# MatchaChoco010/toy-cpu-pathtracing

Measured on AMD Instinct MI355X. Metric: Msamples/sec (whole node), scene3 MIS/Sobol 1920x1080, higher is better.
Workload: dtype f32; 1 GPU; scene3 1920x1080 mis+sobol, 1024-spp job, 1024 sample indices per step (BASELINE configs[1]); parallelism=single-gpu

## Files before the change

include/mi355pt_debug.h:

```cpp
#ifndef MI355PT_DEBUG_H
#define MI355PT_DEBUG_H
#include "mi355pt.h"
#ifdef __cplusplus
extern "C" {
#endif

int mi355pt_debug_unlock(int on);

int mi355pt_scene_debug_set_lowering(mi355pt_scene* s, int mode);

int mi355pt_scene_debug_lowering_digest(const mi355pt_scene* s, const mi355pt_camera* cam, char* names_buf, size_t names_len,
                                        uint64_t* digests, uint32_t* n);

int mi355pt_scene_export_bvh(const mi355pt_scene* s, void* out_nodes, uint32_t* n_nodes, void* out_tris, uint32_t* n_tris,
                             int32_t* root);
int mi355pt_probe_bvh_collapse(const float* tri_pos, uint32_t n_tris, const float* rays_od, uint32_t n_rays, uint32_t* out_info,
                               uint32_t* out_mismatch);
int mi355pt_probe_bvh_collapse_nodes(const void* bvh2_nodes, uint32_t n_nodes, int32_t root, uint32_t n_tris, uint32_t* out_info );
int mi355pt_probe_sobol(uint32_t width, uint32_t height, uint32_t spp, uint32_t seed, const uint32_t* xys ,
                        uint32_t n, const char* pattern, uint32_t* out_bits );
int mi355pt_probe_sincos(uint32_t first_bits, uint32_t stride, uint32_t n, uint64_t* out_counts );
int mi355pt_probe_intersect(const mi355pt_scene* s, const float* origins, const float* dirs, uint32_t n, float* out_t,
                            uint32_t* out_instance, uint32_t* out_triangle, float* out_normal );
int mi355pt_probe_occluded(const mi355pt_scene* s, const float* origins, const float* dirs, const float* t_max, uint32_t n,
                           uint8_t* out_hit);
int mi355pt_sample_log_records(const mi355pt_camera* cam, const mi355pt_params* p, uint32_t sample_begin, uint32_t sample_end,
                               size_t* out_records);
int mi355pt_render_sample_log(const mi355pt_scene* s, const mi355pt_camera* cam, const mi355pt_params* p, uint32_t sample_begin,
                              uint32_t sample_end, float* out_L, float* out_lambda, float* out_pdf, size_t n_records,
                              float* out_accum);
int mi355pt_probe_radiance(const mi355pt_scene* s, const mi355pt_camera* cam, const mi355pt_params* p, const uint32_t* xys,
                           uint32_t n, float* out_L, float* out_lambda, float* out_pdf);


#ifdef __cplusplus
// ... 4 lines not shown
```

toy-cpu-pathtracing_amd/csrc/api.cpp:

```cpp
#include <hip/hip_runtime.h>

#include <algorithm>
#include <cmath>
#include <cstdio>
#include <cstring>
#include <string>
#include <vector>

#include "../../include/mi355pt.h"
#include "api_internal.hpp"

using namespace pt;

static thread_local std::string g_err;
bool pt::g_debug_unlocked = false;
int pt::fail(int code, const std::string& msg) { g_err = msg; return code; }

static const uint32_t CIE_CMF_BITS[470 * 4] = {
#include "cie_cmf.inc"
};
void pt::cie_cmf4(float out[470 * 4]) { std::memcpy(out, CIE_CMF_BITS, sizeof(CIE_CMF_BITS)); }

namespace {

// ... 91 lines not shown
    LaunchCtx* lc; int slot;
    if ((rc = get_launch_ctx(s, p->seed, &lc, &slot))) return rc;
    if (lc->device != s->impl.device) return fail(MI355PT_E_DEVICE, "launch context and scene live on different devices");
    const bool want_stats = stats && p->collect_stats;
    int& waves = aov ? lc->aov_waves[aov_kind] : lc->waves[want_stats ? 1 : 0][p->sampler & 1u][p->strategy < 3u ? p->strategy : 0u];
    if (!waves) waves = aov ? query_resident_waves_aov((uint32_t)aov_kind, s->impl.features)
                            : query_resident_waves(select_kernel(false, want_stats, s->impl.features, p->sampler, p->strategy));
    const DevCamera dc = make_camera(cam);
    LaunchPlan plan = d_list ? plan_launch_tiles(cam, p, s_begin, s_end, waves, n_list) : plan_launch(cam, p, s_begin, s_end, waves, aov);
    DevParams& dp = plan.params;
    if (d_list) set_tile_list(dp, d_list);
    unsigned* d_counter = lc->d_counters + slot;
    DevStats* d_stats = lc->d_stats + slot;
    HIP_TRY(hipMemsetAsync(d_counter, 0, sizeof(unsigned), stream));
    dp.stats_mode = p->collect_stats;
    if (want_stats || (aov && stats)) HIP_TRY(hipMemsetAsync(d_stats, 0, sizeof(DevStats), stream));
    hipEvent_t e0 = nullptr, e1 = nullptr;
    if (stats) { HIP_TRY(hipEventCreate(&e0)); HIP_TRY(hipEventCreate(&e1)); HIP_TRY(hipEventRecord(e0, stream)); }
    if ((rc = grow_device_buffer(&lc->d_partial, &lc->partial_bytes, plan.partial_floats * sizeof(float), stream))) return rc;
    const KernelKey key = select_kernel(d_list != nullptr, want_stats, s->impl.features, p->sampler, p->strategy);
    if ((rc = grow_device_buffer(&lc->d_defer, &lc->defer_bytes, aov ? (size_t)0 : query_defer_bytes_per_wave(key) * (size_t)plan.grid, stream))) return rc;
    if (aov) HIP_TRY(launch_aov((uint32_t)aov_kind, s->impl.dev, dc, dp, illuminant_lut, lc->d_hash, d_accum, d_counter, stats ? d_stats : nullptr,
                                s->impl.features, plan.grid, stream));
    else HIP_TRY(launch_pt(key, s->impl.dev, dc, dp, plan.n_tiles,
                           lc->d_hash, d_accum, lc->d_partial, d_counter, d_list ? nullptr : d_stats, plan.grid, stream, pout, lc->d_defer));
    if (stats) {
        HIP_TRY(hipEventRecord(e1, stream));
        HIP_TRY(hipEventSynchronize(e1));
        float ms = 0.0f;
        HIP_TRY(hipEventElapsedTime(&ms, e0, e1));
        std::memset(stats, 0, sizeof(*stats));
        stats->kernel_ms = ms; stats->launches = 1;
        if (want_stats || aov) {
            DevStats h;
            HIP_TRY(hipMemcpy(&h, d_stats, sizeof(h), hipMemcpyDeviceToHost));
            copy_stats(h, stats);
        }
        (void)hipEventDestroy(e0); (void)hipEventDestroy(e1);
    }
    return MI355PT_OK;
}

static int launch_ranges(const mi355pt_scene* s, const mi355pt_camera* cam, const mi355pt_params* p, uint32_t s_begin, uint32_t s_end, float* d_accum,
                         hipStream_t stream, mi355pt_stats* stats, const uint32_t* d_list, uint32_t n_list,
                         const PathOut& pout = PathOut{nullptr, nullptr, nullptr, 0u, 0u}, int aov_kind = -1, uint32_t illuminant_lut = 0) {
    return for_each_launch_range(p->sampler, stats != nullptr, s_begin, s_end, [&](uint32_t b, uint32_t e) {
        return launch_range(s, cam, p, b, e, d_accum, stream, stats, pout, aov_kind, illuminant_lut, d_list, n_list);
    });
// ... 720 lines not shown
```

toy-cpu-pathtracing_amd/csrc/api_debug.cpp:

```cpp
#include <hip/hip_runtime.h>

#include <algorithm>
#include <cmath>
#include <cstring>
#include <string>
#include <vector>

#include "../../include/mi355pt_debug.h"
#include "api_internal.hpp"
#include "scene_lower.hpp"

using namespace pt;

extern "C" {

int mi355pt_debug_unlock(int on) { const int was = g_debug_unlocked ? 1 : 0; g_debug_unlocked = on != 0; return was; }

int mi355pt_scene_debug_set_lowering(mi355pt_scene* s, int mode) {
    if (!s) return fail(MI355PT_E_INVALID, "null argument");
    if (mode < 0 || mode > 2) return fail(MI355PT_E_INVALID, "unknown lowering mode");
    s->impl.lowering = mode;
    return MI355PT_OK;
}

int mi355pt_scene_debug_lowering_digest(const mi355pt_scene* s, const mi355pt_camera* cam, char* names_buf, size_t names_len, uint64_t* digests, uint32_t* n) {
    if (!s || !cam || !names_buf || !digests || !n) return fail(MI355PT_E_INVALID, "null argument");
    std::string err;
    int rc;
    LoweredGeometry geo; BvhOut bvh; LoweredScene ls; LowerReport rep;
    if ((rc = lower_geometry(s->impl, cam, &geo, &err))) return fail(rc, err);
    build_bvh(geo.build_tris, &bvh);
    if (bvh.max_depth >= STACK_DEPTH) return fail(MI355PT_E_INVALID, "BVH deeper than the traversal stack");
    float cmf[470 * 4];
    cie_cmf4(cmf);
    if ((rc = lower_scene(s->impl, std::move(geo), std::move(bvh), cmf, &ls, &rep, &err)) || (rc = lower_tree4(&ls, &rep, &err))) return fail(rc, err);
    std::vector<std::string> names; std::vector<uint64_t> dig;
    lowering_digests(ls, rep, &names, &dig);
    std::string text;
    for (const std::string& nm : names) text += nm + "\n";
    text += lowering_info(ls, rep, false, nullptr);
    const uint32_t cap = *n;
    *n = (uint32_t)dig.size();
    if (cap < dig.size() || names_len < text.size() + 1) return fail(MI355PT_E_INVALID, "digest or name buffer too small");
    std::memcpy(digests, dig.data(), dig.size() * sizeof(uint64_t));
    std::memcpy(names_buf, text.c_str(), text.size() + 1);
    return MI355PT_OK;
}

int mi355pt_sample_log_records(const mi355pt_camera* cam, const mi355pt_params* p, uint32_t s_begin, uint32_t s_end, size_t* out_records) {
    if (!cam || !p || !out_records || s_end <= s_begin) return fail(MI355PT_E_INVALID, "bad argument");
    *out_records = (size_t)shard_tile_count(cam->width, cam->height, p->shard_index, p->shard_count) * 64u * (s_end - s_begin);
    return MI355PT_OK;
}

int mi355pt_render_sample_log(const mi355pt_scene* s, const mi355pt_camera* cam, const mi355pt_params* p, uint32_t s_begin, uint32_t s_end,
                              float* out_L, float* out_lambda, float* out_pdf, size_t n_records, float* out_accum) {
    int rc = check_args(s, cam, p);
    if (rc) return rc;
    if (!out_L || !out_lambda || !out_pdf || s_end > p->spp || s_begin >= s_end) return fail(MI355PT_E_INVALID, "bad sample range or null output");
    if (p->spp & (p->spp - 1u)) return fail(MI355PT_E_INVALID, "the per-sample log needs a power-of-two spp (the sample index is read back from the Morton index)");
    if (p->collect_stats) return fail(MI355PT_E_INVALID, "the per-sample log is written by the production kernel, not the instrumented one");
    const size_t need = (size_t)shard_tile_count(cam->width, cam->height, p->shard_index, p->shard_count) * 64u * (s_end - s_begin);
    if (n_records != need) return fail(MI355PT_E_INVALID, "n_records must be tiles of the shard * 64 * (sample_end - sample_begin)");
    if (need == 0) return MI355PT_OK;
    const size_t n_film = (size_t)cam->width * cam->height * 3;
    DevBuf<float> d_L, d_lam, d_pdf, d_acc;
    HIP_TRY(d_L.alloc(need * 4)); HIP_TRY(d_lam.alloc(need * 4)); HIP_TRY(d_pdf.alloc(need * 4)); HIP_TRY(d_acc.alloc(n_film));
    HIP_TRY(hipMemset(d_L.p, 0, need * 16)); HIP_TRY(hipMemset(d_lam.p, 0, need * 16)); HIP_TRY(hipMemset(d_pdf.p, 0, need * 16));
// ... 183 lines not shown
```

toy-cpu-pathtracing_amd/csrc/launch_plan.hpp:

```cpp
#pragma once
#include <algorithm>
#include <cmath>
#include <cstddef>
#include <cstdint>
#include <cstdlib>

#include "../../include/mi355pt.h"
#include "layout.hpp"

namespace pt {

struct V3 { float x, y, z; };
inline V3 cross3(V3 a, V3 b) { return {a.y * b.z - b.y * a.z, a.z * b.x - b.z * a.x, a.x * b.y - b.x * a.y}; }
inline V3 norm3(V3 a) { float r = 1.0f / std::sqrt((a.x * a.x) + (a.y * a.y) + (a.z * a.z)); return {a.x * r, a.y * r, a.z * r}; }

inline uint32_t log2_int(uint32_t v) { return v == 0 ? 0 : 31 - (uint32_t)__builtin_clz(v); }
inline uint32_t round_up_pow2(uint32_t v) { return v <= 1 ? 1 : 1u << (32 - __builtin_clz(v - 1)); }

inline uint32_t shard_tile_count(uint32_t width, uint32_t height, uint32_t shard_index, uint32_t shard_count) {
    const uint32_t total = ((width + 7) / 8) * ((height + 7) / 8);
    const uint32_t cnt = shard_count ? shard_count : 1u, idx = shard_count ? shard_index : 0u;
    return total > idx ? (total - idx + cnt - 1) / cnt : 0u;
}

// ... 127 lines not shown
    P(0u) P(FEAT_TEX) P(FEAT_DIEL) P(FEAT_METAL) P(FEAT_DIEL | FEAT_ROUGH) P(FEAT_DELTA | FEAT_MLIGHT) P(FEAT_STD & ~FEAT_CC)           \
    C(FEAT_CC) C(FEAT_CC | FEAT_TEX) C(FEAT_STD) C(FEAT_ALL)
#define PT_NO_SET(F)
#define PT_FOR_EACH_PLAIN_SET(X) PT_FOR_EACH_SET(X, PT_NO_SET)
#define PT_FOR_EACH_CC_SET(X) PT_FOR_EACH_SET(PT_NO_SET, X)
#define PT_SET_ENTRY(F) (F),
inline constexpr uint32_t FEATURE_SETS[] = {PT_FOR_EACH_SET(PT_SET_ENTRY, PT_SET_ENTRY)};
inline constexpr uint32_t PLAIN_SETS[] = {PT_FOR_EACH_PLAIN_SET(PT_SET_ENTRY)};
inline constexpr uint32_t CC_SETS[] = {PT_FOR_EACH_CC_SET(PT_SET_ENTRY)};
#undef PT_SET_ENTRY
inline uint32_t pick_features(uint32_t feat) {
    for (uint32_t s : FEATURE_SETS) if ((feat & ~s) == 0u) return s;
    return FEAT_ALL;
}
struct KernelKey { bool tiles, stats; uint32_t mode, set; };
inline KernelKey select_kernel(bool tiles, bool stats, uint32_t feat, uint32_t sampler, uint32_t strategy) {
    if (stats) return KernelKey{tiles, true, MODE_GENERIC, (feat & (FEAT_CC | FEAT_EMTEX)) == 0u ? FEAT_STD & ~FEAT_CC : FEAT_ALL};
    const uint32_t mode = sampler == MI355PT_SAMPLER_SOBOL && strategy == MI355PT_STRATEGY_MIS ? MODE_MIS_SOBOL
                        : sampler == MI355PT_SAMPLER_SOBOL && strategy == MI355PT_STRATEGY_NEE ? MODE_NEE_SOBOL
                        : strategy == MI355PT_STRATEGY_PT ? MODE_PT : MODE_GENERIC;
    return KernelKey{tiles, false, mode, pick_features(feat)};
}

}
```

toy-cpu-pathtracing_amd/csrc/layout.hpp:

```cpp
#pragma once
#include <stddef.h>
#include <stdint.h>

#if defined(__HIPCC__)
#define PT_HD __host__ __device__
#else
#define PT_HD
#endif

namespace pt {

#ifndef PT_STACK_DEPTH
#define PT_STACK_DEPTH 24
#endif
constexpr int STACK_DEPTH = PT_STACK_DEPTH;
constexpr int MAX_LEAF_TRIS = 4;
constexpr int MAX_BUILD_DEPTH = 22;
constexpr int HASH_TABLE_DIMS = 136;

struct alignas(16) DevNode {
    float bx[4];
    float by[4];
    float bz[4];
    int32_t child[2];
// ... 134 lines not shown
    const DevNode4Q* nodes4q;
    float grid_org[3], grid_cell[3];
    const DevTri* tris;
    const DevTriShade* shade;
    const DevTriLocal* tris_local;
    const DevTri* tris_render;
    float tri_shift[3]; uint32_t tris_are_local;
    float shared_mw[3]; uint32_t pad_mw;
    const DevInstance* instances;
    const DevMaterial* materials;
    const DevLight* lights;
    const DevLightTri* light_tris;
    const float* light_uvs;
    const float* luts;
    const float* cmf;
    const float* rgb2spec;
    const float* z_nodes;
    const uint32_t* texels;
    const DevTexture* textures;
    const float* cc_albedo;
    uint32_t n_nodes, n_tris, n_lights, n_materials;
    int32_t root;
    int32_t root4;
    uint32_t n_nodes4, pad1;
    const DevEnv* envs;
    uint32_t n_envs, pad_env;
};

struct DevCamera {
    float s[3], u[3], f[3];
    float tan_half_fov, aspect;
    uint32_t width, height;
};

struct DevParams {
    uint32_t spp, seed, max_depth, strategy, sampler;
    float exposure;
    uint32_t log2_spp, n_base4_digits;
    uint32_t sample_begin, sample_end;
    uint32_t shard_index, shard_count;
    uint32_t tiles_x, tiles_y;
    uint32_t n_work;
    uint32_t chunks, chunk_size;
    uint32_t block_log2;
    uint32_t sample_prefix_digits;
    uint32_t stats_mode;
    uint32_t albedo_lut;
// ... 23 lines not shown
```

toy-cpu-pathtracing_amd/csrc/pt_kernel.hpp:

```cpp
#pragma once
#include <hip/hip_runtime.h>

#include "launch.hpp"
#include "launch_plan.hpp"
#include "layout.hpp"
#include "pt_device.hpp"
#include "pt_path.hpp"
#include "tail_queue_plan.hpp"

namespace pt {

#ifndef PT_MIN_WAVES_CC
#define PT_MIN_WAVES_CC 3
#endif
#ifndef PT_MIN_WAVES
#define PT_MIN_WAVES 4
#endif
struct LaneJob { uint32_t px, py, s_cur, s_end; bool valid; };
template <typename TileOf>
PT_DEV LaneJob lane_job_at(uint32_t work, uint32_t lane, const DevCamera& cam, const DevParams& prm, TileOf tile_of) {
    LaneJob j{0, 0, 0, 0, false};
    const uint32_t b = prm.block_log2, bside = 1u << b;
    uint32_t item = work / prm.chunks, chunk = work % prm.chunks;
    uint32_t tile_k = item >> (6u - 2u * b), blk = item & ((64u >> (2u * b)) - 1u);
    uint32_t tile = tile_of(tile_k);
    uint32_t tx = tile % prm.tiles_x, ty = tile / prm.tiles_x;
    uint32_t bx = blk & ((8u >> b) - 1u), by = blk >> (3u - b);
    j.px = tx * 8 + bx * bside + (lane & (bside - 1u)); j.py = ty * 8 + by * bside + ((lane >> b) & (bside - 1u));
    j.valid = lane < (1u << (2u * b)) && j.px < cam.width && j.py < cam.height;
    j.s_cur = prm.sample_begin + chunk * prm.chunk_size;
    j.s_end = min(j.s_cur + prm.chunk_size, prm.sample_end);
    return j;
}
// ... 110 lines not shown
```

toy-cpu-pathtracing_amd/csrc/pt_kernel_body.inc:

```
    __shared__ uint32_t s_stack[STACK_DEPTH * 64];
#ifndef PT_FILM_PIX
#define PT_FILM_PIX 64
#endif
    __shared__ float s_film[PT_FILM_PIX * 3];
    __shared__ uint32_t s_hi[SOBOL_HI_DIMS];
    __shared__ uint32_t s_p6[SOBOL_HI_DIMS];
    __shared__ unsigned s_work;
    constexpr bool PARK = (FEAT & FEAT_CC) != 0u && kernel_min_waves<FEAT>() <= 3;
    __shared__ float s_park[PARK ? 8 * 64 : 1];
    __shared__ uint8_t s_perm[96];
    __shared__ uint32_t s_ring[ANY_RING];
    __shared__ uint32_t s_occl[2];
    __shared__ uint32_t s_pair[64];
    const AnyLds any_lds{s_ring, s_occl, s_pair};
    __shared__ unsigned long long s_best[64];
    const ClosestLds closest_lds{s_ring, s_best, s_pair};
    __shared__ uint32_t s_infl[2];
    const PairLds pair_lds{s_ring, s_best, s_occl, s_pair, s_infl};
    DevParams prm = prm_in;
    if constexpr (MODE == MODE_MIS_SOBOL) { prm.strategy = 2u; prm.sampler = 1u; }
    if constexpr (MODE == MODE_NEE_SOBOL) { prm.strategy = 1u; prm.sampler = 1u; }
    if constexpr (MODE == MODE_PT) prm.strategy = 0u;
    const uint32_t lane = threadIdx.x;
    auto park = [&](Path& Q, bool mine = true) {
        if constexpr (PARK) {
            if (mine) {
#pragma unroll
                for (int i = 0; i < 4; ++i) s_park[i * 64 + lane] = Q.pf[i];
                s_park[4 * 64 + lane] = Q.p_pdf; s_park[5 * 64 + lane] = Q.prev_pos.x; s_park[6 * 64 + lane] = Q.prev_pos.y; s_park[7 * 64 + lane] = Q.prev_pos.z;
            }
#pragma unroll
            for (int i = 0; i < 4; ++i) Q.pf[i] = 0.0f;
            Q.p_pdf = 0.0f; Q.prev_pos = mk3(0.0f, 0.0f, 0.0f);
        }
    };
    auto unpark = [&](Path& Q) {
        if constexpr (PARK) {
#pragma unroll
            for (int i = 0; i < 4; ++i) Q.pf[i] = s_park[i * 64 + lane];
            Q.p_pdf = s_park[4 * 64 + lane]; Q.prev_pos = mk3(s_park[5 * 64 + lane], s_park[6 * 64 + lane], s_park[7 * 64 + lane]);
        }
// ... 15 lines not shown
        const uint32_t work = s_work;
        __syncthreads();
        if (work >= prm.n_work) break;
        const LaneJob job = PT_LANE_JOB(work, lane, cam, prm);
        const LaneJob job0 = PT_LANE_JOB(work, 0u, cam, prm);
        const uint32_t blk_log2 = prm.block_log2, blk_mask = (1u << blk_log2) - 1u;
        const uint32_t s_prefix = prm.sample_prefix_digits;
        const uint32_t hi_first_w = sobol_hi_first(prm.log2_spp, blk_log2) - s_prefix, hi_shift_w = 2u * hi_first_w - (prm.log2_spp & 1u);
        if (prm.sampler == 1u && hi_first_w < prm.n_base4_digits && hi_first_w >= 3u &&
            2u * prm.n_base4_digits - (prm.log2_spp & 1u) <= hi_shift_w + 27u) {
            sctx.hi_first = sobol_hi_first(prm.log2_spp, blk_log2) - s_prefix;
            sctx.hi_shift = 2u * sctx.hi_first - (prm.log2_spp & 1u);
            const uint32_t tile_m = (encode_morton2_u32(job0.px, job0.py) << prm.log2_spp) | (s_prefix ? job0.s_cur : 0u);
            for (uint32_t dmn = lane; dmn < (uint32_t)SOBOL_HI_DIMS; dmn += 64) {
                uint32_t e = (uint32_t)(sobol_tile_hi_digits(tile_m, dmn, prm.log2_spp, prm.n_base4_digits, sctx.hi_first) >> sctx.hi_shift);
                const uint64_t prefix = (uint64_t)tile_m >> sctx.hi_shift;
                e |= sobol_perm_index(prefix, dmn) << 27;
                uint32_t e6 = 0;
                for (uint32_t v7 = 0; v7 < 4u; ++v7) e6 |= sobol_perm_index((prefix << 2) | v7, dmn) << (5u * v7);
                s_hi[dmn] = e; s_p6[dmn] = e6;
            }
            sctx.hi_lds = s_hi; sctx.p6_lds = s_p6;
        }
        if (lane < PT_FILM_PIX) { s_film[3 * lane] = 0.0f; s_film[3 * lane + 1] = 0.0f; s_film[3 * lane + 2] = 0.0f; }
        __syncthreads();
        const uint32_t n_s = job0.s_end > job0.s_cur ? job0.s_end - job0.s_cur : 0u;
        const uint32_t pool_size = n_s << (2u * blk_log2);
        uint32_t pool_next = 0u;
        uint32_t my_pix = lane;
        Path P{};
        park(P);
        bool active = false;
        constexpr bool MERGED = merged_traversal<FEAT, MODE>();
        ShadowReq sh{};
        bool dying = false, susp = false;
        CarryState carry{0ull};
        constexpr bool TAILQ = !STATS && tail_queue<FEAT, MODE>();
        constexpr uint32_t DEFER = TAILQ ? 0u : defer_classes<FEAT, MODE>();
        float4* const q_base = (DEFER != 0u || TAILQ) ? defer_buf + (size_t)blockIdx.x * (queue_bytes_per_wave(STATS, FEAT, MODE) / 16u) : nullptr;
        uint32_t q_head = 0u, q_tail = 0u;
        uint32_t q_count = 0u, q2_count = 0u;
        constexpr uint32_t TQ_CLASSES = (TAILQ && (FEAT & FEAT_CC) != 0u) ? ((1u << MT_CLEARCOAT) | (1u << (MT_CLEARCOAT | 8u))) : 0u;
        constexpr uint32_t QR = (TQ_CLASSES != 0u) ? QUEUE_RING : PT_TAILQ_RING1;
        while (true) {
            unsigned long long ts0 = 0, ts1 = 0, ts2 = 0, ts3 = 0, ts4 = 0, tsa = 0, tsb = 0;
            uint32_t bsdf_classes = 0u;
// ... 4 lines not shown
            if (m_needy != 0ull && pool_next < pool_size) {
                const uint32_t idx = pool_next + rank_below(m_needy);
                if (!active && idx < pool_size) {
                    const uint32_t pix = idx & ((1u << (2u * blk_log2)) - 1u);
                    const uint32_t px = job0.px + (pix & blk_mask), py = job0.py + (pix >> blk_log2);
                    const uint32_t smp_i = job0.s_cur + (idx >> (2u * blk_log2));
                    const bool valid = px < cam.width && py < cam.height;
                    if (valid) { active = true; my_pix = pix; regen_path<STATS>(P, sctx, cam, px, py, smp_i, st); }
                }
                pool_next = min(pool_next + (uint32_t)__popcll(m_needy), pool_size);
            }
            if (!__any(active)) {
                if (pool_next >= pool_size && q_tail == q_head && (q_count | q2_count) == 0u) break;
                if (!((DEFER != 0u || TAILQ) && pool_next >= pool_size)) continue;
            }
            if (STATS) { ts1 = __builtin_amdgcn_s_memtime(); if (lane == 0) st.w[4]++; if (active) st.w[5]++; }
            Hit hit{};
            bool got = false;
            const bool canonical = STATS && prm.stats_mode == 1u;
            if (canonical) { if (active) got = trace_closest<STATS>(sc, P.ro, P.rd, 3.402823466e+38f, stack, hit, st); }
            else if constexpr (MERGED) {
                bool occluded = false;
                if (STATS && sh.on) st.w[6]++;
                PT_PRIO_TRAV_ENTER;
                trace_pair_coop<STATS>(sc, P.ro, P.rd, active && !dying && !popped, sh.o, sh.d, sh.t, sh.on, stack, lane, pair_lds, hit, got, occluded, st, &carry, susp, &susp);
                PT_PRIO_TRAV_EXIT;
                if (sh.on && !occluded) {
#pragma unroll
                    for (int i = 0; i < 4; ++i) P.L[i] = P.L[i] + sh.c[i];
                }
                sh = ShadowReq{};
            }
            else { PT_PRIO_TRAV_ENTER; got = trace_closest_coop<STATS>(sc, P.ro, P.rd, active, stack, lane, closest_lds, hit, st); PT_PRIO_TRAV_EXIT; }
            if (STATS) {
                const uint32_t mclass = (active && got) ? sc.materials[__float_as_uint(((const float4*)(sc.shade + hit.tri))[4].z)].type : 8u;
                uint32_t classes = 0u, largest = 0u, lanes = 0u;
                for (uint32_t c = 0u; c < 8u; ++c) {
                    const uint32_t n = (uint32_t)__popcll(__ballot(mclass == c));
                    classes += n ? 1u : 0u; largest = max(largest, n); lanes += n;
                }
                if (lane == 0 && lanes) { st.dv[0]++; st.dv[1] += classes; st.dv[2] += lanes; st.dv[3] += largest; }
                bsdf_classes = classes - (__ballot(mclass == MT_EMISSIVE) != 0ull ? 1u : 0u);
                ts2 = __builtin_amdgcn_s_memtime();
            }
            auto tq_store = [&](uint32_t e, const Path& Q, const Hit& h, uint32_t pix) {
                float4* r = q_base + (size_t)(e >> 8) * (TQ_F4 * QUEUE_RING) + (e & (QR - 1u));
                const uint32_t fl = (Q.wl.term ? 1u : 0u) | ((Q.depth & 1023u) << 1) | ((pix & 63u) << 11) | (Q.smp.dimension << 17);
                r[0u * QR] = make_float4(__uint_as_float(Q.smp.morton), __uint_as_float(fl), Q.wl.lam0, __uint_as_float(h.tri));
                r[1u * QR] = make_float4(Q.T[0], Q.T[1], Q.T[2], Q.T[3]);
// ... 233 lines not shown
```

toy-cpu-pathtracing_amd/csrc/scene_lower.cpp:

```cpp
#include "scene_lower.hpp"

#include <algorithm>
#include <cfloat>
#include <cmath>
#include <cstdio>
#include <cstring>

namespace pt {

namespace {

constexpr float PI_F = 3.14159265358979323846f;

struct V3 { float x, y, z; };
inline V3 operator-(V3 a, V3 b) { return {a.x - b.x, a.y - b.y, a.z - b.z}; }
inline V3 cross(V3 a, V3 b) { return {a.y * b.z - b.y * a.z, a.z * b.x - b.z * a.x, a.x * b.y - b.x * a.y}; }
inline float dot(V3 a, V3 b) { return (a.x * b.x) + (a.y * b.y) + (a.z * b.z); }
inline float length(V3 a) { return std::sqrt(dot(a, a)); }
inline V3 normalize(V3 a) { float r = 1.0f / length(a); return {a.x * r, a.y * r, a.z * r}; }
inline V3 vertex(const HostMesh& mesh, uint32_t v) { return V3{mesh.pos[3 * v], mesh.pos[3 * v + 1], mesh.pos[3 * v + 2]}; }
inline bool degenerate(V3 a, V3 b, V3 c) { const V3 cr = cross(b - a, c - a); return dot(cr, cr) == 0.0f; }

template <typename Rec>
inline void set_vertices(Rec& r, V3 a, V3 b, V3 c) {
// ... 577 lines not shown
           " depth=" + std::to_string(rep.bvh_depth) + " builder=" + (gpu_builder ? "gpu" : "host") + t_bvh + " collapse=" + rep.collapse_method + t_collapse + tail;
}

void lowering_digests(const LoweredScene& ls, const LowerReport& rep, std::vector<std::string>* names, std::vector<uint64_t>* digests) {
    names->clear(); digests->clear();
    auto add = [&](const std::string& name, const void* p, size_t bytes) { names->push_back(name); digests->push_back(fnv1a64(p, bytes)); };
#define PT_DIGEST(v) add(#v, ls.v.data(), ls.v.size() * sizeof(ls.v[0]))
    PT_DIGEST(nodes); PT_DIGEST(nodes4); PT_DIGEST(tris_render); PT_DIGEST(shade); PT_DIGEST(instances); PT_DIGEST(tris_local); PT_DIGEST(cc_albedo);
    PT_DIGEST(materials); PT_DIGEST(lights); PT_DIGEST(light_tris); PT_DIGEST(light_uvs); PT_DIGEST(luts); PT_DIGEST(cmf); PT_DIGEST(rgb2spec);
    PT_DIGEST(z_nodes); PT_DIGEST(texels); PT_DIGEST(textures);
#undef PT_DIGEST
    for (size_t k = 0; k < ls.env_tables.size(); ++k) {
        const LoweredScene::EnvTables& t = ls.env_tables[k];
        const std::string e = "env" + std::to_string(k);
        add(e + ".texels", t.texels.data(), t.texels.size() * 4); add(e + ".marginal", t.marginal.data(), t.marginal.size() * 4);
        add(e + ".conditional", t.conditional.data(), t.conditional.size() * 4);
    }
    add("envs", ls.envs.data(), ls.envs.size() * sizeof(DevEnv));
    std::string b;
    auto put = [&](const void* p, size_t n) { b.append((const char*)p, n); };
    const DevScene& dev = ls.dev;
    put(dev.grid_org, 12); put(dev.grid_cell, 12); put(dev.tri_shift, 12); put(&dev.tris_are_local, 4); put(dev.shared_mw, 12); put(&dev.pad_mw, 4);
    put(&dev.n_nodes, 4); put(&dev.n_tris, 4); put(&dev.n_lights, 4); put(&dev.n_materials, 4); put(&dev.root, 4); put(&dev.root4, 4);
    put(&dev.n_nodes4, 4); put(&dev.pad1, 4); put(&dev.n_envs, 4); put(&dev.pad_env, 4);
    const uint32_t feat = ls.features; const uint64_t ndeg = rep.n_degenerate, nn4 = dev.n_nodes4; const int32_t depth = rep.bvh_depth, need = rep.stack_need;
    put(&feat, 4); put(&ndeg, 8); put(&depth, 4); put(&nn4, 8); put(&need, 4); put(rep.collapse_method, std::strlen(rep.collapse_method));
    add("scalars", b.data(), b.size());
}

}
```

toy-cpu-pathtracing_amd/ffi.py:

```python
import ctypes as C
import os

import numpy as np

HERE = os.path.dirname(os.path.abspath(__file__))
ROOT = os.path.dirname(HERE)
LIB_PATH = os.environ.get("MI355PT_LIB") or os.path.join(HERE, "csrc", "libmi355pt.so")

NONE = 0xFFFFFFFF
SPEC_CONSTANT, SPEC_RGB_ALBEDO_SRGB, SPEC_LUT470, SPEC_TEXTURE_ALBEDO_SRGB, SPEC_SIGMOID, SPEC_RGB_ALBEDO_SRGB_LINEAR = 0, 1, 2, 3, 4, 5
SPEC_TEXTURE_ILLUMINANT_SRGB, SPEC_TEXTURE_UNBOUNDED_SRGB = 6, 7
MAT_LAMBERT, MAT_EMISSIVE, MAT_GLASS, MAT_PLASTIC, MAT_CLEARCOAT, MAT_METAL, MAT_SIMPLE_PBR = 0, 1, 2, 3, 4, 5, 6
STRATEGY = {"pt": 0, "nee": 1, "mis": 2}
SAMPLER = {"random": 0, "sobol": 1}
AOV_NORMAL, AOV_ALBEDO, AOV_SHADING_NORMAL = 0, 1, 2
AOV = {"normal": AOV_NORMAL, "albedo": AOV_ALBEDO, "shading_normal": AOV_SHADING_NORMAL}


class Spectrum(C.Structure):
    _fields_ = [("kind", C.c_uint32), ("id", C.c_uint32), ("c", C.c_float * 3)]

    @staticmethod
    def constant(v):
        return Spectrum(SPEC_CONSTANT, 0, (C.c_float * 3)(v, 0, 0))
# ... 120 lines not shown


class UpsampleGuides(C.Structure):
    _fields_ = [("albedo", C.c_void_p), ("shading_normal", C.c_void_p), ("position", C.c_void_p), ("hit", C.c_void_p)]


UPSAMPLE_GUIDES = ("albedo", "shading_normal", "position", "hit")


def make_camera(position, direction, up, width, height, fov_deg=45.0):
    return Camera((C.c_float * 3)(*position), (C.c_float * 3)(*direction), (C.c_float * 3)(*up), fov_deg, width, height)


def make_params(spp, strategy="mis", sampler="sobol", seed=0, max_depth=16, exposure=1.0, shard_index=0, shard_count=1,
                collect_stats=0, rr_gate_slack=0.0, albedo_lut=0):
    return Params(spp, seed, max_depth, STRATEGY[strategy], SAMPLER[sampler], exposure, shard_index, shard_count, collect_stats, rr_gate_slack,
                  albedo_lut)


def _ptr(a, ty):
    return a.ctypes.data_as(C.POINTER(ty)) if a is not None else None


DEBUG_SYMBOLS = ["debug_unlock", "scene_debug_set_lowering", "scene_debug_lowering_digest", "scene_export_bvh", "probe_bvh_collapse", "probe_bvh_collapse_nodes", "probe_sobol", "probe_sincos", "probe_intersect", "probe_occluded",
                 "sample_log_records", "render_sample_log", "probe_radiance"]
ABI_SYMBOLS = [
    "scene_create", "scene_destroy", "scene_set_rgb2spec", "scene_add_lut470", "scene_add_tex_rgb8", "scene_add_mesh",
    "scene_add_material", "scene_add_instance", "scene_add_delta_light", "scene_add_environment_light", "scene_set_bvh_builder", "scene_build", "render", "render_accum_device", "film_resolve_device",
    "render_accum_tiles_device",
    "render_aov", "render_aov_accum_device", "aov_resolve_device",
    "quantize_u8", "scene_info", "scene_build_multi", "render_multi", "coat_albedo_table",
    "last_error", "version",
]
DENOISE_SYMBOLS = ["denoise_params_default", "denoise_scratch_bytes", "denoise_device", "denoise"]
DENOISE_VAR_SYMBOLS = ["denoise_var_params_default", "denoise_var_scratch_bytes", "denoise_var_device", "denoise_var"]
GBUFFER_SYMBOLS = ["render_gbuffer_accum_device", "gbuffer_normalize_device", "render_gbuffer"]
TEMPORAL_SYMBOLS = ["temporal_params_default", "temporal_view_from_cameras", "temporal_accumulate_device", "temporal_accumulate"]
TEMPORAL_RECTIFY_SYMBOLS = ["temporal_rectify_params_default", "temporal_rectify_scratch_bytes", "temporal_accumulate_rectified_device",
                            "temporal_accumulate_rectified"]
UPSAMPLE_SYMBOLS = ["upsample_params_default", "upsample_low_camera", "upsample_device", "upsample"]
ADAPTIVE_SYMBOLS = ["adaptive_scratch_bytes", "adaptive_step_device", "film_normalize_tiles_device", "render_adaptive_device", "render_adaptive"]


class Backend:

    def __init__(self, lib, prefix):
        self.lib, self.prefix = lib, prefix
# ... 132 lines not shown
        m = np.eye(4, dtype=np.float32) if local_to_world is None else np.asarray(local_to_world, dtype=np.float32)
        cols = np.ascontiguousarray(m.T.reshape(-1))
        self.b.check(self.b.fn("scene_add_environment_light")(self.h, intensity, _ptr(rgb, C.c_float), rgb.shape[1], rgb.shape[0],
                                                              _ptr(cols, C.c_float), illuminant_lut), "scene_add_environment_light")

    def set_bvh_builder(self, mode):
        fn = self.b.fn("scene_set_bvh_builder")
        fn.argtypes = [C.c_void_p, C.c_int]
        self.b.check(fn(self.h, {"auto": 0, "host": 1, "gpu": 2}[mode]), "scene_set_bvh_builder")

    def debug_set_lowering(self, mode):
        fn = self.b.fn("scene_debug_set_lowering")
        fn.argtypes = [C.c_void_p, C.c_int]
        self.b.check(fn(self.h, {"auto": 0, "no_local_tris": 1, "general": 2}[mode]), "scene_debug_set_lowering")

    def debug_lowering_digest(self, cam):
        fn = self.b.fn("scene_debug_lowering_digest")
        fn.argtypes = [C.c_void_p, C.POINTER(Camera), C.c_char_p, C.c_size_t, C.POINTER(C.c_uint64), C.POINTER(C.c_uint32)]
        text = C.create_string_buffer(4096); dig = (C.c_uint64 * 128)(); n = C.c_uint32(128)
        self.b.check(fn(self.h, C.byref(cam), text, 4096, dig, C.byref(n)), "scene_debug_lowering_digest")
        *names, info = text.value.decode().split("\n")
        assert len(names) == n.value
        return {nm: f"{dig[i]:016x}" for i, nm in enumerate(names)}, info

    def build(self, cam):
        self.b.check(self.b.fn("scene_build")(self.h, C.byref(cam)), "scene_build")

    def probe_intersect(self, origins, dirs):
        o = np.ascontiguousarray(origins, dtype=np.float32).reshape(-1, 3)
        d = np.ascontiguousarray(dirs, dtype=np.float32).reshape(-1, 3)
        n = o.shape[0]
        t = np.zeros(n, np.float32); inst = np.zeros(n, np.uint32); tri = np.zeros(n, np.uint32); nrm = np.zeros((n, 3), np.float32)
        self.b.check(self.b.fn("probe_intersect")(self.h, _ptr(o, C.c_float), _ptr(d, C.c_float), n, _ptr(t, C.c_float),
                                                   _ptr(inst, C.c_uint32), _ptr(tri, C.c_uint32), _ptr(nrm, C.c_float)), "probe_intersect")
        return t, inst, tri, nrm

    def probe_occluded(self, origins, dirs, t_max):
        o = np.ascontiguousarray(origins, dtype=np.float32).reshape(-1, 3)
        d = np.ascontiguousarray(dirs, dtype=np.float32).reshape(-1, 3)
        tm = np.ascontiguousarray(t_max, dtype=np.float32).reshape(-1)
        out = np.zeros(o.shape[0], np.uint8)
        self.b.check(self.b.fn("probe_occluded")(self.h, _ptr(o, C.c_float), _ptr(d, C.c_float), _ptr(tm, C.c_float), o.shape[0],
                                                  _ptr(out, C.c_uint8)), "probe_occluded")
        return out

    def probe_radiance(self, cam, params, xys):
# ... 400 lines not shown
```

Measured before the change: 2628 Msamples/s.

## Cull per-block candidate triangle lists for primary camera rays via frustum walk

```diff
diff --git a/include/mi355pt_debug.h b/include/mi355pt_debug.h
--- a/include/mi355pt_debug.h
+++ b/include/mi355pt_debug.h
@@ -11,6 +11,9 @@
 
 int mi355pt_scene_debug_lowering_digest(const mi355pt_scene* s, const mi355pt_camera* cam, char* names_buf, size_t names_len,
                                         uint64_t* digests, uint32_t* n);
+
+int mi355pt_scene_debug_camera_candidates(const mi355pt_scene* s, const mi355pt_camera* cam, const uint32_t* rects, uint32_t n_rects, uint32_t cap,
+                                          uint32_t* out_counts, uint8_t* out_overflow, uint32_t* out_indices, float* out_tris, uint32_t* n_tris);
 
 int mi355pt_scene_export_bvh(const mi355pt_scene* s, void* out_nodes, uint32_t* n_nodes, void* out_tris, uint32_t* n_tris,
                              int32_t* root);
diff --git a/toy-cpu-pathtracing_amd/csrc/api.cpp b/toy-cpu-pathtracing_amd/csrc/api.cpp
--- a/toy-cpu-pathtracing_amd/csrc/api.cpp
+++ b/toy-cpu-pathtracing_amd/csrc/api.cpp
@@ -137,8 +137,12 @@
     if ((rc = grow_device_buffer(&lc->d_defer, &lc->defer_bytes, aov ? (size_t)0 : query_defer_bytes_per_wave(key) * (size_t)plan.grid, stream))) return rc;
     if (aov) HIP_TRY(launch_aov((uint32_t)aov_kind, s->impl.dev, dc, dp, illuminant_lut, lc->d_hash, d_accum, d_counter, stats ? d_stats : nullptr,
                                 s->impl.features, plan.grid, stream));
-    else HIP_TRY(launch_pt(key, s->impl.dev, dc, dp, plan.n_tiles,
-                           lc->d_hash, d_accum, lc->d_partial, d_counter, d_list ? nullptr : d_stats, plan.grid, stream, pout, lc->d_defer));
+    else {
+        DevScene dev = s->impl.dev;
+        dev.cam_lists = use_camera_lists(key, dp.block_log2, camera_lists_enabled()) ? 1u : 0u;
+        HIP_TRY(launch_pt(key, dev, dc, dp, plan.n_tiles,
+                          lc->d_hash, d_accum, lc->d_partial, d_counter, d_list ? nullptr : d_stats, plan.grid, stream, pout, lc->d_defer));
+    }
     if (stats) {
         HIP_TRY(hipEventRecord(e1, stream));
         HIP_TRY(hipEventSynchronize(e1));
diff --git a/toy-cpu-pathtracing_amd/csrc/api_debug.cpp b/toy-cpu-pathtracing_amd/csrc/api_debug.cpp
--- a/toy-cpu-pathtracing_amd/csrc/api_debug.cpp
+++ b/toy-cpu-pathtracing_amd/csrc/api_debug.cpp
@@ -8,6 +8,7 @@
 
 #include "../../include/mi355pt_debug.h"
 #include "api_internal.hpp"
+#include "camera_candidates.hpp"
 #include "scene_lower.hpp"
 
 using namespace pt;
@@ -44,6 +45,41 @@
     if (cap < dig.size() || names_len < text.size() + 1) return fail(MI355PT_E_INVALID, "digest or name buffer too small");
     std::memcpy(digests, dig.data(), dig.size() * sizeof(uint64_t));
     std::memcpy(names_buf, text.c_str(), text.size() + 1);
+    return MI355PT_OK;
+}
+
+int mi355pt_scene_debug_camera_candidates(const mi355pt_scene* s, const mi355pt_camera* cam, const uint32_t* rects, uint32_t n_rects, uint32_t cap,
+                                          uint32_t* out_counts, uint8_t* out_overflow, uint32_t* out_indices, float* out_tris, uint32_t* n_tris) {
+    if (!s || !cam || (n_rects && (!rects || !out_counts || !out_overflow))) return fail(MI355PT_E_INVALID, "null argument");
+    if (cap < 1u || cap > 4096u) return fail(MI355PT_E_INVALID, "cap must be 1 .. 4096");
+    if (PT_NODE_Q16) return fail(MI355PT_E_INVALID, "the candidate walk reads the float 4-wide tree");
+    std::string err;
+    int rc;
+    LoweredGeometry geo; BvhOut bvh; LoweredScene ls; LowerReport rep;
+    if ((rc = lower_geometry(s->impl, cam, &geo, &err))) return fail(rc, err);
+    build_bvh(geo.build_tris, &bvh);
+    if (bvh.max_depth >= STACK_DEPTH) return fail(MI355PT_E_INVALID, "BVH deeper than the traversal stack");
+    float cmf[470 * 4];
+    cie_cmf4(cmf);
+    if ((rc = lower_scene(s->impl, std::move(geo), std::move(bvh), cmf, &ls, &rep, &err)) || (rc = lower_tree4(&ls, &rep, &err))) return fail(rc, err);
+    const uint32_t n = (uint32_t)ls.tris_render.size();
+    if (out_tris) {
+        if (!n_tris || *n_tris < n) return fail(MI355PT_E_INVALID, "triangle buffer too small");
+        for (uint32_t i = 0; i < n; ++i) std::memcpy(out_tris + 9 * (size_t)i, &ls.tris_render[i], 9 * sizeof(float));
+    }
+    if (n_tris) *n_tris = n;
+#if !PT_NODE_Q16
+    const DevCamera dc = make_camera(cam);
+    const DevTri* tris = ls.dev.tris_are_local ? ls.tris_local.data() : ls.tris_render.data();
+    uint32_t stack[CAM_WALK_STACK];
+    std::vector<uint32_t> list(cap);
+    for (uint32_t r = 0; r < n_rects; ++r) {
+        const uint32_t* q = rects + 4 * (size_t)r;
+        const CamWalk w = cam_walk(ls.nodes4.data(), ls.dev.root4, tris, ls.dev.tri_shift, cam_pyramid(dc, q[0], q[1], q[2], q[3]), list.data(), cap, stack);
+        out_counts[r] = w.count; out_overflow[r] = w.overflow ? 1 : 0;
+        if (out_indices) std::memcpy(out_indices + (size_t)r * cap, list.data(), sizeof(uint32_t) * w.count);
+    }
+#endif
     return MI355PT_OK;
 }
 
diff --git a/toy-cpu-pathtracing_amd/csrc/camera_candidates.hpp b/toy-cpu-pathtracing_amd/csrc/camera_candidates.hpp
--- /dev/null
+++ b/toy-cpu-pathtracing_amd/csrc/camera_candidates.hpp
@@ -0,0 +1,115 @@
+#pragma once
+#include <cstdint>
+
+#include "layout.hpp"
+
+#ifndef PT_CAM_UNIFORM
+#define PT_CAM_UNIFORM(v) (v)
+#endif
+
+namespace pt {
+
+constexpr float CAM_MARGIN_PIX = 0.125f;
+constexpr float CAM_SLACK_REL = 1.0f / (float)(1u << 20);
+constexpr uint32_t CAM_LIST_CAP = 16u;
+constexpr uint32_t CAM_WALK_STACK = 96u;
+
+struct CamPyramid { float n[5][3]; float n1[5]; };
+
+PT_HD inline float cam_abs(float v) { return v < 0.0f ? -v : v; }
+PT_HD inline float cam_min(float a, float b) { return a < b ? a : b; }
+PT_HD inline float cam_max(float a, float b) { return a < b ? b : a; }
+
+PT_HD inline CamPyramid cam_pyramid(const DevCamera& cam, uint32_t x0, uint32_t y0, uint32_t x1, uint32_t y1) {
+    const float fx_lo = (float)x0 - CAM_MARGIN_PIX, fx_hi = (float)x1 + 1.0f + CAM_MARGIN_PIX;
+    const float fy_lo = (float)y0 - CAM_MARGIN_PIX, fy_hi = (float)y1 + 1.0f + CAM_MARGIN_PIX;
+    const float dx_lo = (2.0f * fx_lo / (float)cam.width - 1.0f) * cam.aspect * cam.tan_half_fov;
+    const float dx_hi = (2.0f * fx_hi / (float)cam.width - 1.0f) * cam.aspect * cam.tan_half_fov;
+    const float dy_hi = (1.0f - 2.0f * fy_lo / (float)cam.height) * cam.tan_half_fov;
+    const float dy_lo = (1.0f - 2.0f * fy_hi / (float)cam.height) * cam.tan_half_fov;
+    CamPyramid py;
+    for (int a = 0; a < 3; ++a) {
+        py.n[0][a] = cam.s[a] - dx_hi * cam.f[a];
+        py.n[1][a] = dx_lo * cam.f[a] - cam.s[a];
+        py.n[2][a] = cam.u[a] - dy_hi * cam.f[a];
+        py.n[3][a] = dy_lo * cam.f[a] - cam.u[a];
+        py.n[4][a] = -cam.f[a];
+    }
+    for (int k = 0; k < 5; ++k) py.n1[k] = cam_abs(py.n[k][0]) + cam_abs(py.n[k][1]) + cam_abs(py.n[k][2]);
+    return py;
+}
+
+PT_HD inline bool cam_box_outside(const CamPyramid& py, const float lo[3], const float hi[3], float extent) {
+    bool outside = false;
+    for (int k = 0; k < 5; ++k) {
+        const float m = cam_min(py.n[k][0] * lo[0], py.n[k][0] * hi[0]) + cam_min(py.n[k][1] * lo[1], py.n[k][1] * hi[1]) +
+                        cam_min(py.n[k][2] * lo[2], py.n[k][2] * hi[2]);
+        outside = outside || m > CAM_SLACK_REL * py.n1[k] * extent;
+    }
+    return outside;
+}
+
+PT_HD inline bool cam_slot_used(const DevNode4& nd, int c) { return nd.lox[c] <= nd.hix[c] && nd.lox[c] < 3.402823466e+38f; }
+
+PT_HD inline float cam_tree_extent(const DevNode4* nodes, int32_t root4) {
+    float r = 0.0f;
+    if (root4 < 0) return r;
+    const DevNode4& nd = nodes[root4];
+    for (int c = 0; c < 4; ++c) {
+        if (!cam_slot_used(nd, c)) continue;
+        r = cam_max(r, cam_max(cam_max(cam_abs(nd.lox[c]), cam_abs(nd.hix[c])), cam_max(cam_abs(nd.loy[c]), cam_abs(nd.hiy[c]))));
+        r = cam_max(r, cam_max(cam_abs(nd.loz[c]), cam_abs(nd.hiz[c])));
+    }
+    return r;
+}
+
+struct CamWalk { uint32_t count; bool overflow; };
+
+PT_HD inline CamWalk cam_walk(const DevNode4* nodes, int32_t root4, const DevTri* tris, const float tri_shift[3], const CamPyramid& py, uint32_t* out,
+                              uint32_t cap, uint32_t* stack) {
+    CamWalk w{0u, false};
+    const float extent = cam_tree_extent(nodes, root4);
+    const float extent_tri = extent + cam_max(cam_max(cam_abs(tri_shift[0]), cam_abs(tri_shift[1])), cam_abs(tri_shift[2]));
+    uint32_t sp = 0u;
+    int32_t cur = root4;
+    for (;;) {
+        if (cur < 0) {
+            const uint32_t first = leaf_first(cur), cnt = leaf_count(cur);
+            for (uint32_t base = 0; base < cnt; base += 4u) {
+                DevTri t[4];
+                for (uint32_t i = 0; i < 4u; ++i) t[i] = tris[first + (base + i < cnt ? base + i : cnt - 1u)];
+                bool keep[4];
+                for (uint32_t i = 0; i < 4u; ++i) {
+                    const float v[3][3] = {{t[i].p0[0], t[i].p0[1], t[i].p0[2]}, {t[i].p1x, t[i].p1yz[0], t[i].p1yz[1]}, {t[i].p2xy[0], t[i].p2xy[1], t[i].p2z}};
+                    float lo[3], hi[3];
+                    for (int a = 0; a < 3; ++a) {
+                        lo[a] = cam_min(cam_min(v[0][a], v[1][a]), v[2][a]) - tri_shift[a];
+                        hi[a] = cam_max(cam_max(v[0][a], v[1][a]), v[2][a]) - tri_shift[a];
+                    }
+                    keep[i] = base + i < cnt && !cam_box_outside(py, lo, hi, extent_tri);
+                }
+                for (uint32_t i = 0; i < 4u; ++i) {
+                    if (!keep[i]) continue;
+                    if (w.count >= cap) { w.overflow = true; return w; }
+                    out[w.count++] = first + base + i;
+                }
+            }
+        } else {
+            const DevNode4 nd = nodes[cur];
+            bool keep[4];
+            for (int c = 0; c < 4; ++c) {
+                const float lo[3] = {nd.lox[c], nd.loy[c], nd.loz[c]}, hi[3] = {nd.hix[c], nd.hiy[c], nd.hiz[c]};
+                keep[c] = cam_slot_used(nd, c) && !cam_box_outside(py, lo, hi, extent);
+            }
+            for (int c = 0; c < 4; ++c) {
+                if (!keep[c]) continue;
+                if (sp >= CAM_WALK_STACK) { w.overflow = true; return w; }
+                stack[sp++] = (uint32_t)nd.child[c];
+            }
+        }
+        if (sp == 0u) return w;
+        cur = (int32_t)PT_CAM_UNIFORM(stack[--sp]);
+    }
+}
+
+}
diff --git a/toy-cpu-pathtracing_amd/csrc/launch_plan.hpp b/toy-cpu-pathtracing_amd/csrc/launch_plan.hpp
--- a/toy-cpu-pathtracing_amd/csrc/launch_plan.hpp
+++ b/toy-cpu-pathtracing_amd/csrc/launch_plan.hpp
@@ -173,4 +173,7 @@
     return KernelKey{tiles, false, mode, pick_features(feat)};
 }
 
+inline bool use_camera_lists(const KernelKey& key, uint32_t block_log2, bool enabled) { return enabled && !key.stats && block_log2 <= 3u; }
+inline bool camera_lists_enabled() { const char* e = getenv("MI355PT_NO_CAMERA_LISTS"); return !(e && e[0] != '\0' && !(e[0] == '0' && e[1] == '\0')); }
+
 }
diff --git a/toy-cpu-pathtracing_amd/csrc/layout.hpp b/toy-cpu-pathtracing_amd/csrc/layout.hpp
--- a/toy-cpu-pathtracing_amd/csrc/layout.hpp
+++ b/toy-cpu-pathtracing_amd/csrc/layout.hpp
@@ -180,7 +180,8 @@
     uint32_t n_nodes, n_tris, n_lights, n_materials;
     int32_t root;
     int32_t root4;
-    uint32_t n_nodes4, pad1;
+    uint32_t n_nodes4;
+    uint32_t cam_lists;
     const DevEnv* envs;
     uint32_t n_envs, pad_env;
 };
diff --git a/toy-cpu-pathtracing_amd/csrc/pt_kernel.hpp b/toy-cpu-pathtracing_amd/csrc/pt_kernel.hpp
--- a/toy-cpu-pathtracing_amd/csrc/pt_kernel.hpp
+++ b/toy-cpu-pathtracing_amd/csrc/pt_kernel.hpp
@@ -7,8 +7,12 @@
 #include "pt_device.hpp"
 #include "pt_path.hpp"
 #include "tail_queue_plan.hpp"
+#define PT_CAM_UNIFORM(v) ((uint32_t)__builtin_amdgcn_readfirstlane((int)(v)))
+#include "camera_candidates.hpp"
 
 namespace pt {
+
+constexpr uint32_t CAM_LIST_NONE = 0xffffffffu;
 
 #ifndef PT_MIN_WAVES_CC
 #define PT_MIN_WAVES_CC 3
diff --git a/toy-cpu-pathtracing_amd/csrc/pt_kernel_body.inc b/toy-cpu-pathtracing_amd/csrc/pt_kernel_body.inc
--- a/toy-cpu-pathtracing_amd/csrc/pt_kernel_body.inc
+++ b/toy-cpu-pathtracing_amd/csrc/pt_kernel_body.inc
@@ -17,6 +17,8 @@
     const ClosestLds closest_lds{s_ring, s_best, s_pair};
     __shared__ uint32_t s_infl[2];
     const PairLds pair_lds{s_ring, s_best, s_occl, s_pair, s_infl};
+    constexpr bool CAMLIST = !STATS && tail_queue<FEAT, MODE>();
+    __shared__ uint32_t s_cand[CAMLIST ? CAM_LIST_CAP : 1u];
     DevParams prm = prm_in;
     if constexpr (MODE == MODE_MIS_SOBOL) { prm.strategy = 2u; prm.sampler = 1u; }
     if constexpr (MODE == MODE_NEE_SOBOL) { prm.strategy = 1u; prm.sampler = 1u; }
@@ -78,6 +80,14 @@
             }
             sctx.hi_lds = s_hi; sctx.p6_lds = s_p6;
         }
+        uint32_t cam_n = CAM_LIST_NONE;
+        if constexpr (CAMLIST) {
+            if (sc.cam_lists != 0u) {
+                const uint32_t x0 = PT_CAM_UNIFORM(job0.px), y0 = PT_CAM_UNIFORM(job0.py);
+                const CamWalk cw = cam_walk(sc.nodes4, sc.root4, sc.tris, sc.tri_shift, cam_pyramid(cam, x0, y0, x0 + blk_mask, y0 + blk_mask), s_cand, CAM_LIST_CAP, s_ring);
+                cam_n = PT_CAM_UNIFORM(cw.overflow ? CAM_LIST_NONE : cw.count);
+            }
+        }
         if (lane < PT_FILM_PIX) { s_film[3 * lane] = 0.0f; s_film[3 * lane + 1] = 0.0f; s_film[3 * lane + 2] = 0.0f; }
         __syncthreads();
         const uint32_t n_s = job0.s_end > job0.s_cur ? job0.s_end - job0.s_cur : 0u;
@@ -128,9 +138,33 @@
             else if constexpr (MERGED) {
                 bool occluded = false;
                 if (STATS && sh.on) st.w[6]++;
-                PT_PRIO_TRAV_ENTER;
-                trace_pair_coop<STATS>(sc, P.ro, P.rd, active && !dying && !popped, sh.o, sh.d, sh.t, sh.on, stack, lane, pair_lds, hit, got, occluded, st, &carry, susp, &susp);
-                PT_PRIO_TRAV_EXIT;
+                bool cam_ray = false;
+                if constexpr (CAMLIST) cam_ray = cam_n != CAM_LIST_NONE && active && !dying && P.from_camera && P.depth == 0u;
+                if (!CAMLIST || __ballot((active && !dying && !popped && !cam_ray) || sh.on) != 0ull) {
+                    PT_PRIO_TRAV_ENTER;
+                    trace_pair_coop<STATS>(sc, P.ro, P.rd, active && !dying && !popped && !cam_ray, sh.o, sh.d, sh.t, sh.on, stack, lane, pair_lds, hit, got, occluded, st, &carry, susp, &susp);
+                    PT_PRIO_TRAV_EXIT;
+                }
+                if constexpr (CAMLIST) {
+                    if (__ballot(cam_ray) != 0ull) {
+                        const RaySetup rs = setup_ray(P.rd);
+                        const f3 o2 = tri_origin(sc, P.ro);
+                        unsigned long long key = (0x7f7fffffull << 32) | 0xffffffffull;
+                        for (uint32_t i = 0u; i < cam_n; ++i) {
+                            const uint32_t tri = PT_CAM_UNIFORM(s_cand[i]);
+                            const TriVerts tv = load_tri(sc.tris, tri);
+                            float t, b0, b1, b2;
+                            if (intersect_triangle<false>(o2, P.rd, rs.kx, rs.ky, rs.kz, rs.sx, rs.sy, rs.sz, 3.402823466e+38f, tv, t, b0, b1, b2)) {
+                                const unsigned long long k = ((unsigned long long)__float_as_uint(t) << 32) | (unsigned long long)tri;
+                                key = k < key ? k : key;
+                            }
+                        }
+                        if (cam_ray) {
+                            got = (uint32_t)key != 0xffffffffu;
+                            if (got) winner_hit(sc, P.ro, P.rd, rs, (uint32_t)key, hit);
+                        }
+                    }
+                }
                 if (sh.on && !occluded) {
 #pragma unroll
                     for (int i = 0; i < 4; ++i) P.L[i] = P.L[i] + sh.c[i];
diff --git a/toy-cpu-pathtracing_amd/csrc/scene_lower.cpp b/toy-cpu-pathtracing_amd/csrc/scene_lower.cpp
--- a/toy-cpu-pathtracing_amd/csrc/scene_lower.cpp
+++ b/toy-cpu-pathtracing_amd/csrc/scene_lower.cpp
@@ -623,7 +623,7 @@
     const DevScene& dev = ls.dev;
     put(dev.grid_org, 12); put(dev.grid_cell, 12); put(dev.tri_shift, 12); put(&dev.tris_are_local, 4); put(dev.shared_mw, 12); put(&dev.pad_mw, 4);
     put(&dev.n_nodes, 4); put(&dev.n_tris, 4); put(&dev.n_lights, 4); put(&dev.n_materials, 4); put(&dev.root, 4); put(&dev.root4, 4);
-    put(&dev.n_nodes4, 4); put(&dev.pad1, 4); put(&dev.n_envs, 4); put(&dev.pad_env, 4);
+    put(&dev.n_nodes4, 4); put(&dev.cam_lists, 4); put(&dev.n_envs, 4); put(&dev.pad_env, 4);
     const uint32_t feat = ls.features; const uint64_t ndeg = rep.n_degenerate, nn4 = dev.n_nodes4; const int32_t depth = rep.bvh_depth, need = rep.stack_need;
     put(&feat, 4); put(&ndeg, 8); put(&depth, 4); put(&nn4, 8); put(&need, 4); put(rep.collapse_method, std::strlen(rep.collapse_method));
     add("scalars", b.data(), b.size());
diff --git a/toy-cpu-pathtracing_amd/ffi.py b/toy-cpu-pathtracing_amd/ffi.py
--- a/toy-cpu-pathtracing_amd/ffi.py
+++ b/toy-cpu-pathtracing_amd/ffi.py
@@ -166,7 +166,7 @@
     return a.ctypes.data_as(C.POINTER(ty)) if a is not None else None
 
 
-DEBUG_SYMBOLS = ["debug_unlock", "scene_debug_set_lowering", "scene_debug_lowering_digest", "scene_export_bvh", "probe_bvh_collapse", "probe_bvh_collapse_nodes", "probe_sobol", "probe_sincos", "probe_intersect", "probe_occluded",
+DEBUG_SYMBOLS = ["debug_unlock", "scene_debug_set_lowering", "scene_debug_lowering_digest", "scene_debug_camera_candidates", "scene_export_bvh", "probe_bvh_collapse", "probe_bvh_collapse_nodes", "probe_sobol", "probe_sincos", "probe_intersect", "probe_occluded",
                  "sample_log_records", "render_sample_log", "probe_radiance"]
 ABI_SYMBOLS = [
     "scene_create", "scene_destroy", "scene_set_rgb2spec", "scene_add_lut470", "scene_add_tex_rgb8", "scene_add_mesh",
@@ -345,6 +345,22 @@
         *names, info = text.value.decode().split("\n")
         assert len(names) == n.value
         return {nm: f"{dig[i]:016x}" for i, nm in enumerate(names)}, info
+
+    def debug_camera_candidates(self, cam, rects, cap=16, want_tris=False):
+        fn = self.b.fn("scene_debug_camera_candidates")
+        fn.argtypes = [C.c_void_p, C.POINTER(Camera), C.POINTER(C.c_uint32), C.c_uint32, C.c_uint32, C.POINTER(C.c_uint32), C.POINTER(C.c_uint8),
+                       C.POINTER(C.c_uint32), C.POINTER(C.c_float), C.POINTER(C.c_uint32)]
+        r = np.ascontiguousarray(rects, dtype=np.uint32).reshape(-1, 4)
+        n = r.shape[0]
+        counts = np.zeros(n, np.uint32); over = np.zeros(n, np.uint8); idx = np.zeros((n, cap), np.uint32)
+        nt = C.c_uint32(0)
+        tris = None
+        if want_tris:
+            self.b.check(fn(self.h, C.byref(cam), None, 0, cap, None, None, None, None, C.byref(nt)), "scene_debug_camera_candidates")
+            tris = np.zeros((nt.value, 3, 3), np.float32)
+        self.b.check(fn(self.h, C.byref(cam), _ptr(r, C.c_uint32), n, cap, _ptr(counts, C.c_uint32), _ptr(over, C.c_uint8), _ptr(idx, C.c_uint32),
+                        _ptr(tris, C.c_float), C.byref(nt)), "scene_debug_camera_candidates")
+        return (counts, over.astype(bool), idx, tris) if want_tris else (counts, over.astype(bool), idx)
 
     def build(self, cam):
         self.b.check(self.b.fn("scene_build")(self.h, C.byref(cam)), "scene_build")
```

New measurement: 2695 Msamples/s, median of 6. 2.6% higher.
